# LeoIV/polyaxon

Hardware: AMD Instinct MI355X
Metric: HPO trials/hour (whole node) + wall-clock-to-target, ResNet-50 Hyperband sweep (higher is better)
Workload: dtype bf16

## Files before the change

polyaxon_amd/csrc/conv_gemm.hip:

```cpp
#include <hip/hip_runtime.h>

#include <stdint.h>

#include <type_traits>

namespace {

typedef __bf16 bf16x8 __attribute__((ext_vector_type(8)));
typedef short s16x4 __attribute__((ext_vector_type(4)));
typedef float f32x4 __attribute__((ext_vector_type(4)));
typedef uint32_t u32x4 __attribute__((ext_vector_type(4)));
typedef __attribute__((address_space(3))) void lds_void;
typedef __attribute__((address_space(1))) const void gbl_void;

constexpr int BK = 64;

struct ConvGeom {
    int H, W;
    int Hr, Wr;
    int C, S, ntaps;
    int Hc, Wc, OS, oph, opw;
    signed char offh[9], offw[9], btap[9];
    int tap_a[9], tap_b[9];
    uint32_t mWr, mHr;
// ... 24 lines not shown
        while (j < g.nw && g.wv[j] != g.offw[t]) ++j;
        if (j == g.nw) g.wv[g.nw++] = g.offw[t];
        g.pat[i * 3 + j] |= 1u << t;
    }
    g.mWr = div_magic(g.Wr);
    g.mHr = div_magic(g.Hr);
    return g;
}

struct BnBwd {
    const __bf16* x;
    const uint8_t* mask;
    const float* mean;
    const float* invstd;
    float* part;
    int part_ld, blk_off;
    int skip_h, skip_w;
};

struct BnDx {
    const __bf16* x;
    const uint8_t* mask;
    const float* coef;
    __bf16* dy;
};

struct BnApply {
    const __bf16* res;
    const float* sb;
    const float* rsb;
    __bf16* out;
    uint8_t* mask;
};

__device__ __forceinline__ void row_coords(int m, int Hr, int Wr, int& n, int& r, int& c) {
    const int q = m / Wr;
    c = m - q * Wr;
    n = q / Hr;
    r = q - n * Hr;
}

__device__ __forceinline__ void row_coords(int m, const ConvGeom& g, int& n, int& r, int& c) {
    const int q = g.mWr ? (int)__umulhi((uint32_t)m, g.mWr) : m;
    c = m - q * g.Wr;
    n = g.mHr ? (int)__umulhi((uint32_t)q, g.mHr) : q;
    r = q - n * g.Hr;
}

__device__ __forceinline__ size_t out_row(const ConvGeom& g, int m) {
    if (g.OS == 0) return (size_t)m;
    int n, r, c;
    row_coords(m, g.Hr, g.Wr, n, r, c);
    return ((size_t)n * g.Hc + r * g.OS + g.oph) * g.Wc + c * g.OS + g.opw;
}
constexpr int NTHREADS = 256;

template <int STEP>
__device__ __forceinline__ void wait_vm_stages(int stages) {
    if (stages >= 4 && 4 * STEP <= 63) asm volatile("s_waitcnt vmcnt(%0)" ::"n"(4 * STEP < 63 ? 4 * STEP : 63) : "memory");
    else if (stages >= 3) asm volatile("s_waitcnt vmcnt(%0)" ::"n"(3 * STEP) : "memory");
    else if (stages == 2) asm volatile("s_waitcnt vmcnt(%0)" ::"n"(2 * STEP) : "memory");
    else if (stages == 1) asm volatile("s_waitcnt vmcnt(%0)" ::"n"(STEP) : "memory");
    else asm volatile("s_waitcnt vmcnt(0)" ::: "memory");
}

__device__ __forceinline__ int xcd_remap(int bid, int nwg) {
    const int xcd = bid & 7, q = nwg >> 3, r = nwg & 7;
    const int base = xcd < r ? xcd * (q + 1) : r * (q + 1) + (xcd - r) * q;
    return base + (bid >> 3);
}

__device__ __forceinline__ void glds16(const void* g, void* l) {
    __builtin_amdgcn_global_load_lds((gbl_void*)g, (lds_void*)l, 16, 0, 0);
}

constexpr uint32_t OOB = 0x80000000u;

__device__ __forceinline__ __amdgpu_buffer_rsrc_t buf_rsrc(const void* base) {
    return __builtin_amdgcn_make_buffer_rsrc(const_cast<void*>(base), 0, (int)OOB, 0x00020000);
}

__device__ __forceinline__ void blds16(__amdgpu_buffer_rsrc_t r, uint32_t off, void* l) {
    __builtin_amdgcn_raw_ptr_buffer_load_lds(r, (lds_void*)l, 16, off, 0, 0, 0);
}

__device__ __forceinline__ uint32_t pack_bf16x2(float a, float b) {
    return (uint32_t)__builtin_bit_cast(uint16_t, (__bf16)a) | ((uint32_t)__builtin_bit_cast(uint16_t, (__bf16)b) << 16);
}

__device__ __forceinline__ int nt_swz(int row) { return (row >> 1) & 7; }

template <int BM, int BN, int WGM, int WGN, int MODE, int MINB = 2, int NBUF = 2, bool BWD = false, int NTH = NTHREADS,
          bool BNDX = false, int BNAP = 0>
__global__ void __launch_bounds__(NTH, MINB)
gemm_nt_kernel(const __bf16* __restrict__ A, const __bf16* __restrict__ B, __bf16* __restrict__ C,
               int M, int N, int K, int lda, int ldb, int ldc, float* __restrict__ stats, ConvGeom geo,
               const __bf16* __restrict__ D, int ldd, BnBwd bnr, const uint8_t* __restrict__ dmask, BnDx bd,
               BnApply ba) {
    constexpr bool CONV = MODE == 1, STEM = MODE == 2;
    constexpr bool PROD = BNDX || BNAP != 0;
    static_assert(BNAP >= 0 && BNAP <= 2 && !(BNDX && BNAP != 0), "one producer mode");
    static_assert(BNAP == 0 || (MODE == 0 && NBUF == 2 && !BWD && NTH == 256), "BNAP: dense double-buffered forward");
    static_assert(MODE >= 0 && MODE <= 2, "dense, gather or stem");
    static_assert(!BNDX || (MODE == 0 && NBUF == 2 && BWD && NTH == 256), "BNDX: dense double-buffered data gradient");
    constexpr int NW = NTH / 64;
    static_assert(WGM * WGN == NW, "one wave per wave tile");
    static_assert(NTH == 256 && NBUF >= 1 && NBUF <= 2, "4-wave kernels, one or two K stages");
    constexpr int WTM = BM / WGM, WTN = BN / WGN;
    constexpr int RM = WTM / 16, RN = WTN / 16;
    constexpr int A_BYTES = BM * BK * 2, B_BYTES = BN * BK * 2, STAGE = A_BYTES + B_BYTES;
    extern __shared__ __attribute__((aligned(16))) char smem[];

    const int tid = threadIdx.x, lane = tid & 63;
    const int wave = __builtin_amdgcn_readfirstlane(tid >> 6);
    const int ntn = N / BN, ntm = (M + BM - 1) / BM;
    const int id = xcd_remap(blockIdx.x, ntm * ntn);
    const int tn = id % ntn, tm = id / ntn;
    const int m0 = tm * BM, n0 = tn * BN;
    const int wm = wave / WGN, wn = wave % WGN;

    constexpr int AI = BM / (8 * NW), BI = BN / (8 * NW);
    int a_off[AI];
    uint32_t a_ok[AI];
#pragma unroll
    for (int i = 0; i < AI; ++i) {
        const int row = (i * NW + wave) * 8 + (lane >> 3);
        const int lc = (lane & 7) ^ nt_swz(row);
        const int gm = m0 + row;
        if constexpr (CONV) {
            int n, r, c;
            row_coords(gm, geo, n, r, c);
            const int ih0 = r * geo.S, iw0 = c * geo.S;
            a_off[i] = (((n * geo.H + ih0) * geo.W + iw0) * lda + lc * 8) * 2;
            uint32_t ok = 0;
#pragma unroll
            for (int hi = 0; hi < 3; ++hi) {
                const bool vh = hi < geo.nh && (unsigned)(ih0 + geo.hv[hi]) < (unsigned)geo.H;
#pragma unroll
                for (int wj = 0; wj < 3; ++wj) {
                    const bool vw = wj < geo.nw && (unsigned)(iw0 + geo.wv[wj]) < (unsigned)geo.W;
                    ok |= (vh && vw) ? geo.pat[hi * 3 + wj] : 0u;
                }
            }
            a_ok[i] = gm < M ? ok : 0u;
        } else if constexpr (STEM) {
            int n, r, c;
            row_coords(gm, geo, n, r, c);
            const int ih0 = 2 * r - 3, sc0 = c - 2;
            a_off[i] = ((n * geo.H + ih0) * geo.W + sc0) * 16;
            uint32_t ok = 0;
#pragma unroll
            for (int st = 0; st < 4; ++st) {
                const int t = st * 8 + lc;
                ok |= (t < 28 && (unsigned)(ih0 + (t >> 2)) < (unsigned)geo.H && (unsigned)(sc0 + (t & 3)) < (unsigned)geo.W)
                          ? 1u << st : 0u;
            }
            a_ok[i] = gm < M ? ok : 0u;
        } else {
            a_off[i] = (gm * lda + lc * 8) * 2;
            a_ok[i] = gm < M ? 1u : 0u;
        }
    }
    int b_off[BI];
#pragma unroll
    for (int i = 0; i < BI; ++i) {
        const int row = (i * NW + wave) * 8 + (lane >> 3);
// ... 813 lines not shown
        if (it + R2 < nu) issue(it + R2);
    }
    if (!lag) __builtin_amdgcn_s_barrier();
    asm volatile("s_waitcnt vmcnt(0) lgkmcnt(0)" ::: "memory");
    __syncthreads();
    float* red = (float*)smem;
    if (grp > 0) {
        float* dst = red + ((grp - 1) * GW + wg) * 4096 + lane;
#pragma unroll
        for (int a = 0; a < 4; ++a)
#pragma unroll
            for (int b = 0; b < 4; ++b)
#pragma unroll
                for (int r = 0; r < 4; ++r) dst[((a * 4 + b) * 4 + r) * 64] = acc[a][b][r];
    }
    __syncthreads();
    if (!ATOMIC && grp > 0) return;
    if (grp == 0) {
#pragma unroll 1
        for (int g = 1; g < KS; ++g) {
            const float* src = red + ((g - 1) * GW + wg) * 4096 + lane;
#pragma unroll
            for (int a = 0; a < 4; ++a)
#pragma unroll
                for (int b = 0; b < 4; ++b)
#pragma unroll
                    for (int r = 0; r < 4; ++r) acc[a][b][r] += src[((a * 4 + b) * 4 + r) * 64];
        }
    }
    if constexpr (ATOMIC) {
        __syncthreads();
        if (grp == 0) {
            float* t = red + wg * 4096;
#pragma unroll
            for (int a = 0; a < 4; ++a)
#pragma unroll
                for (int b = 0; b < 4; ++b)
#pragma unroll
                    for (int r = 0; r < 4; ++r) {
                        const int row = a * 16 + 4 * g4 + r, col = b * 16 + gi;
                        t[row * 64 + (col ^ (((row >> 2) & 3) << 4))] = acc[a][b][r];
                    }
        }
        __syncthreads();
#pragma unroll 4
        for (int j = wave; j < GW * 64; j += NW) {
            const int tw = j >> 6, row = j & 63;
            const float v = red[tw * 4096 + row * 64 + (lane ^ (((row >> 2) & 3) << 4))];
            float* dst = W + (size_t)(n10 + (tw / NB) * 64 + row) * ldc + n20 + (tw % NB) * 64 + lane;
            __hip_atomic_fetch_add(dst, v, __ATOMIC_RELAXED, __HIP_MEMORY_SCOPE_AGENT);
        }
        return;
    }
    float* slab = W + (size_t)slice * N1 * N2;
#pragma unroll
    for (int a = 0; a < 4; ++a)
#pragma unroll
        for (int b = 0; b < 4; ++b) {
            const int c2 = n20 + w2 * 64 + b * 16 + gi;
            const int r1 = n10 + w1 * 64 + a * 16 + 4 * g4;
#pragma unroll
            for (int r = 0; r < 4; ++r) slab[(size_t)(r1 + r) * N2 + c2] = acc[a][b][r];
        }
}

__global__ void weight_prep_kernel(const float* __restrict__ w, __bf16* __restrict__ wb, __bf16* __restrict__ wt,
                                   int cout, int cin) {
    __shared__ float tile[32][33];
    const int c0 = blockIdx.x * 32, o0 = blockIdx.y * 32;
    const int tx = threadIdx.x & 31, ty = threadIdx.x >> 5;
    for (int j = ty; j < 32; j += 8) {
        const int o = o0 + j, c = c0 + tx;
        float v = (o < cout && c < cin) ? w[(size_t)o * cin + c] : 0.f;
        tile[j][tx] = v;
        if (o < cout && c < cin) wb[(size_t)o * cin + c] = (__bf16)v;
    }
    __syncthreads();
    for (int j = ty; j < 32; j += 8) {
        const int c = c0 + j, o = o0 + tx;
        if (o < cout && c < cin) wt[(size_t)c * cout + o] = (__bf16)tile[tx][j];
    }
}

template <int NK>
__global__ void __launch_bounds__(512, 1)
bndx_wgrad_kernel(const __bf16* __restrict__ G, const __bf16* __restrict__ B, __bf16* __restrict__ C, int M, int ldb,
                  int ldc, const __bf16* __restrict__ D, int ldd, BnBwd bnr, const uint8_t* __restrict__ dmask, BnDx bd,
                  const __bf16* __restrict__ Xin, float* __restrict__ dW, int lddw) {
    constexpr int BM = 256, BN = 64, NW = 8, K = NK * BK;
    constexpr int A_BYTES = BM * BK * 2, B_BYTES = BN * BK * 2, STAGE = A_BYTES + B_BYTES;
    constexpr int XOFF = 2 * STAGE;
    constexpr int AI = BM / (8 * NW);
    extern __shared__ __attribute__((aligned(16))) char smem[];

    const int ntm = (M + BM - 1) / BM;
    if ((int)blockIdx.x >= ntm) return;
    const int tid = threadIdx.x, lane = tid & 63;
    const int wave = __builtin_amdgcn_readfirstlane(tid >> 6);
    const int fr = lane & 15, fq = lane >> 4;

    const int srow = wave * 8 + (lane >> 3);
    const int lc8 = ((lane & 7) ^ tr_swz<128>(srow)) * 8;
    const uint32_t b_off = (uint32_t)((srow * ldb + ((lane & 7) ^ nt_swz(srow)) * 8) * 2);
    const __amdgpu_buffer_rsrc_t rg = buf_rsrc(G), rb = buf_rsrc(B), rx = buf_rsrc(bd.x), rc = buf_rsrc(bd.coef),
                                 rxi = buf_rsrc(Xin);
    uint32_t e_off[AI];
    u32x4 gq[AI], xq[AI];
    uint32_t mq[AI];
    u32x4 cf[6];
    auto set_tile = [&](int m0) {
#pragma unroll
        for (int i = 0; i < AI; ++i) {
            const int gm = m0 + i * 64 + srow;
            e_off[i] = gm < M ? (uint32_t)((gm * K + lc8) * 2) : OOB;
        }
    };
    auto stage_x = [&](int m0) {
#pragma unroll
        for (int i = 0; i < AI; ++i) {
            const int gm = m0 + i * 64 + srow;
            blds16(rxi, gm < M ? (uint32_t)((gm * BN + lc8) * 2) : OOB, smem + XOFF + (i * NW + wave) * 1024);
        }
    };
    auto stage_b = [&](int buf, int k0) { blds16(rb, b_off + (uint32_t)(k0 * 2), smem + buf * STAGE + A_BYTES + wave * 1024); };
    auto load_a = [&](int k0) {
#pragma unroll
        for (int i = 0; i < AI; ++i) {
            gq[i] = __builtin_amdgcn_raw_buffer_load_b128(rg, (int)e_off[i], k0 * 2, 0);
            xq[i] = __builtin_amdgcn_raw_buffer_load_b128(rx, (int)e_off[i], k0 * 2, 0);
        }
        if (bd.mask != nullptr) {
            const __amdgpu_buffer_rsrc_t rm = buf_rsrc(bd.mask);
#pragma unroll
            for (int i = 0; i < AI; ++i)
                mq[i] = __builtin_amdgcn_raw_buffer_load_b8(rm, (int)(e_off[i] == OOB ? OOB : e_off[i] >> 4), k0 >> 3, 0);
        } else {
#pragma unroll
            for (int i = 0; i < AI; ++i) mq[i] = 0xffu;
        }
#pragma unroll
        for (int r = 0; r < 3; ++r) {
            cf[2 * r] = __builtin_amdgcn_raw_buffer_load_b128(rc, lc8 * 4, (r * K + k0) * 4, 0);
            cf[2 * r + 1] = __builtin_amdgcn_raw_buffer_load_b128(rc, lc8 * 4 + 16, (r * K + k0) * 4, 0);
        }
    };
    auto xform_a = [&](int buf) {
        char* base = smem + buf * STAGE;
        const float* ca = (const float*)&cf[0];
        const float* cb = (const float*)&cf[2];
        const float* cd = (const float*)&cf[4];
#pragma unroll
        for (int i = 0; i < AI; ++i) {
            const uint32_t* pg = (const uint32_t*)&gq[i];
            const uint32_t* px = (const uint32_t*)&xq[i];
            u32x4 o;
            uint32_t* po = (uint32_t*)&o;
            const uint32_t mb = mq[i];
#pragma unroll
            for (int j = 0; j < 4; ++j) {
                const float g0 = (mb >> (2 * j)) & 1u ? __uint_as_float(pg[j] << 16) : 0.f;
                const float g1 = (mb >> (2 * j + 1)) & 1u ? __uint_as_float(pg[j] & 0xffff0000u) : 0.f;
                const float x0 = __uint_as_float(px[j] << 16), x1 = __uint_as_float(px[j] & 0xffff0000u);
                const float o0 = fmaf(ca[2 * j], g0, fmaf(cb[2 * j], x0, cd[2 * j]));
                const float o1 = fmaf(ca[2 * j + 1], g1, fmaf(cb[2 * j + 1], x1, cd[2 * j + 1]));
                po[j] = pack_bf16x2(o0, o1);
            }
            if (e_off[i] == OOB) o = u32x4{0u, 0u, 0u, 0u};
            *(u32x4*)(base + (i * NW + wave) * 1024 + lane * 16) = o;
        }
    };

    f32x4 accw[NK][2];
#pragma unroll
    for (int a = 0; a < NK; ++a) accw[a][0] = accw[a][1] = f32x4{0.f, 0.f, 0.f, 0.f};
    const int kt4 = wave >> 1, nt2 = (wave & 1) * 2;
    const int trow = 8 * fq + (fr >> 2), tcol = 4 * (fr & 3);
    auto tr_off = [&](int col) {
        return (uint32_t)(trow * 128 + (((col >> 3) ^ tr_swz<128>(trow)) << 4) + ((col >> 2) & 1) * 8);
    };
    const uint32_t wa_off = tr_off(kt4 * 16 + tcol), wx_off0 = tr_off(nt2 * 16 + tcol), wx_off1 = tr_off(nt2 * 16 + 16 + tcol);

    constexpr int CROW = BN * 2 + 16, CHUNKS = BN / 8, RSTEP = 256 / CHUNKS, ITERS = BM / RSTEP;
    char* const ep = smem + STAGE;
    const bool bnr_on = bnr.part != nullptr, d_on = D != nullptr;

    int tm = blockIdx.x;
    set_tile(tm * BM);
    stage_x(tm * BM);
    load_a(0);
    stage_b(0, 0);
    for (; tm < ntm; tm += gridDim.x) {
        const int m0 = tm * BM;
        f32x4 acc[4][2];
#pragma unroll
        for (int a = 0; a < 4; ++a) acc[a][0] = acc[a][1] = f32x4{0.f, 0.f, 0.f, 0.f};
        xform_a(0);
        asm volatile("s_waitcnt vmcnt(0)" ::: "memory");
        __syncthreads();
#pragma unroll
        for (int kt = 0; kt < NK; ++kt) {
            const int cur = kt & 1;
            if (kt + 1 < NK) {
                load_a((kt + 1) * BK);
                stage_b(cur ^ 1, (kt + 1) * BK);
            }
            const char* As = smem + cur * STAGE;
            const char* Bs = As + A_BYTES;
#pragma unroll
            for (int kk = 0; kk < 2; ++kk) {
                bf16x8 fa[4], fb[2];
#pragma unroll
                for (int rn = 0; rn < 4; ++rn) {
                    const int row = rn * 16 + fr;
                    fa[rn] = *(const bf16x8*)(Bs + row * 128 + (((kk * 4 + fq) ^ nt_swz(row)) << 4));
                }
#pragma unroll
                for (int rm = 0; rm < 2; ++rm) {
                    const int row = wave * 32 + rm * 16 + fr;
                    fb[rm] = *(const bf16x8*)(As + row * 128 + (((kk * 4 + fq) ^ tr_swz<128>(row)) << 4));
                }
#pragma unroll
                for (int rn = 0; rn < 4; ++rn)
#pragma unroll
                    for (int rm = 0; rm < 2; ++rm)
                        acc[rn][rm] = __builtin_amdgcn_mfma_f32_16x16x32_bf16(fa[rn], fb[rm], acc[rn][rm], 0, 0, 0);
            }
            const uint32_t sa_ = lds_addr(As) + wa_off;
            const uint32_t sx_[2] = {lds_addr(smem + XOFF) + wx_off0, lds_addr(smem + XOFF) + wx_off1};
            auto dw_steps = [&](auto msc) {
                constexpr int O = decltype(msc)::value * 32 * 128;
                s16x4 alo[2], ahi[2], xlo[2][2], xhi[2][2];
                alo[0] = ds_tr_o<O>(sa_);
                ahi[0] = ds_tr_o<O + 512>(sa_);
                alo[1] = ds_tr_o<O + 4096>(sa_);
                ahi[1] = ds_tr_o<O + 4608>(sa_);
#pragma unroll
                for (int j = 0; j < 2; ++j) {
                    xlo[0][j] = ds_tr_o<O>(sx_[j]);
                    xhi[0][j] = ds_tr_o<O + 512>(sx_[j]);
                    xlo[1][j] = ds_tr_o<O + 4096>(sx_[j]);
                    xhi[1][j] = ds_tr_o<O + 4608>(sx_[j]);
                }
                asm volatile("s_waitcnt lgkmcnt(0)"
                             : "+v"(alo[0]), "+v"(ahi[0]), "+v"(alo[1]), "+v"(ahi[1]), "+v"(xlo[0][0]), "+v"(xhi[0][0]),
                               "+v"(xlo[0][1]), "+v"(xhi[0][1]), "+v"(xlo[1][0]), "+v"(xhi[1][0]), "+v"(xlo[1][1]),
                               "+v"(xhi[1][1]));
#pragma unroll
                for (int u = 0; u < 2; ++u) {
                    const bf16x8 fw = __builtin_bit_cast(bf16x8, __builtin_shufflevector(alo[u], ahi[u], 0, 1, 2, 3, 4, 5, 6, 7));
#pragma unroll
                    for (int j = 0; j < 2; ++j) {
                        const bf16x8 fx =
                            __builtin_bit_cast(bf16x8, __builtin_shufflevector(xlo[u][j], xhi[u][j], 0, 1, 2, 3, 4, 5, 6, 7));
                        accw[kt][j] = __builtin_amdgcn_mfma_f32_16x16x32_bf16(fw, fx, accw[kt][j], 0, 0, 0);
                    }
                }
            };
            dw_steps(std::integral_constant<int, 0>{});
            dw_steps(std::integral_constant<int, 2>{});
            dw_steps(std::integral_constant<int, 4>{});
            dw_steps(std::integral_constant<int, 6>{});
            __builtin_amdgcn_sched_barrier(0);
            if (kt + 1 < NK) xform_a(cur ^ 1);
            asm volatile("s_waitcnt vmcnt(0)" ::: "memory");
            __syncthreads();
        }
        const int tnext = tm + gridDim.x;
        if (tnext < ntm) {
            set_tile(tnext * BM);
            stage_x(tnext * BM);
            load_a(0);
            stage_b(0, 0);
        }
        const int rows = min(BM, M - m0);
        int te = tid;
        asm volatile("" : "+v"(te));
        const int cc = te % CHUNKS, ch0 = cc * 8;
        const bool ep_thread = te < 256;
#pragma unroll
        for (int rm = 0; rm < 2; ++rm) {
            const int ml = wave * 32 + rm * 16 + fr;
#pragma unroll
            for (int rn = 0; rn < 4; ++rn) {
                const f32x4 v = acc[rn][rm];
                uint2 packed;
                packed.x = pack_bf16x2(v[0], v[1]);
                packed.y = pack_bf16x2(v[2], v[3]);
                *(uint2*)(ep + ml * CROW + (rn * 16 + fq * 4) * 2) = packed;
            }
        }
        __syncthreads();
        {
            constexpr int AIT = BM / 64;
            const int ra0 = te / CHUNKS;
            int orow[AIT];
            uint4 dpre[AIT];
            uint32_t dmpre[AIT];
#pragma unroll
            for (int i = 0; i < AIT; ++i) orow[i] = min(m0 + ra0 + i * 64, M - 1);
            if (d_on) {
#pragma unroll
                for (int i = 0; i < AIT; ++i) dpre[i] = *(const uint4*)(D + (size_t)orow[i] * ldd + ch0);
                if (dmask != nullptr) {
#pragma unroll
                    for (int i = 0; i < AIT; ++i) dmpre[i] = dmask[((size_t)orow[i] * ldd + ch0) >> 3];
                }
            }
#pragma unroll
            for (int i = 0; i < AIT; ++i) {
                const int r = ra0 + i * 64;
                if (r >= rows) break;
                uint4 v = *(const uint4*)(ep + r * CROW + cc * 16);
                if (d_on) {
                    uint32_t* pv = (uint32_t*)&v;
                    const uint32_t* pd = (const uint32_t*)&dpre[i];
                    const uint32_t db = dmask != nullptr ? dmpre[i] : 0xffu;
#pragma unroll
                    for (int j = 0; j < 4; ++j) {
                        const float d0 = (db >> (2 * j)) & 1u ? __uint_as_float(pd[j] << 16) : 0.f;
                        const float d1 = (db >> (2 * j + 1)) & 1u ? __uint_as_float(pd[j] & 0xffff0000u) : 0.f;
                        const float lo = __uint_as_float(pv[j] << 16) + d0;
                        const float hi = __uint_as_float(pv[j] & 0xffff0000u) + d1;
                        pv[j] = pack_bf16x2(lo, hi);
                    }
                    if (bnr_on) *(uint4*)(ep + r * CROW + cc * 16) = v;
                }
                *(uint4*)(C + (size_t)orow[i] * ldc + ch0) = v;
            }
        }
        float sa[8], sb[8];
        if (bnr_on) {
            __syncthreads();
            if (ep_thread) {
                const int r0 = te / CHUNKS;
                float mu[8], is[8];
#pragma unroll
                for (int k = 0; k < 8; ++k) {
                    sa[k] = sb[k] = 0.f;
                    mu[k] = bnr.mean[ch0 + k];
                    is[k] = bnr.invstd[ch0 + k];
                }
#pragma unroll
                for (int h = 0; h < 2; ++h) {
                    constexpr int HI = ITERS / 2;
                    asm volatile("" ::: "memory");
                    uint4 xpre[HI];
                    uint32_t mpre[HI];
#pragma unroll
                    for (int i = 0; i < HI; ++i) {
                        const size_t e = (size_t)min(m0 + r0 + (h * HI + i) * RSTEP, M - 1) * ldc + ch0;
                        xpre[i] = *(const uint4*)(bnr.x + e);
                        mpre[i] = bnr.mask != nullptr ? bnr.mask[e >> 3] : 0xffu;
                    }
                    if (bnr.skip_w > 0) {
#pragma unroll
                        for (int i = 0; i < HI; ++i) {
                            const int gm = m0 + r0 + (h * HI + i) * RSTEP, q = gm / bnr.skip_w;
                            if (((gm - q * bnr.skip_w) | (q % bnr.skip_h)) % 2 == 0) mpre[i] = 0u;
                        }
                    }
#pragma unroll
                    for (int i = 0; i < HI; ++i) {
                        const int r = r0 + (h * HI + i) * RSTEP;
                        if (r >= rows) break;
                        const uint4 v = *(const uint4*)(ep + r * CROW + cc * 16);
                        const uint32_t mb = mpre[i];
                        const uint32_t* pv = (const uint32_t*)&v;
                        const uint32_t* px = (const uint32_t*)&xpre[i];
#pragma unroll
                        for (int j = 0; j < 4; ++j) {
                            const float g0 = (mb >> (2 * j)) & 1u ? __uint_as_float(pv[j] << 16) : 0.f;
                            const float g1 = (mb >> (2 * j + 1)) & 1u ? __uint_as_float(pv[j] & 0xffff0000u) : 0.f;
                            const float x0 = __uint_as_float(px[j] << 16), x1 = __uint_as_float(px[j] & 0xffff0000u);
                            sa[2 * j] += g0;
                            sa[2 * j + 1] += g1;
                            sb[2 * j] = fmaf(g0, (x0 - mu[2 * j]) * is[2 * j], sb[2 * j]);
                            sb[2 * j + 1] = fmaf(g1, (x1 - mu[2 * j + 1]) * is[2 * j + 1], sb[2 * j + 1]);
                        }
                    }
                }
            }
        }
        if (bnr_on) {
            float* red = (float*)ep;
            __syncthreads();
            if (ep_thread) {
#pragma unroll
                for (int k = 0; k < 8; ++k) {
                    red[te * 17 + k] = sa[k];
                    red[te * 17 + 8 + k] = sb[k];
                }
            }
            __syncthreads();
            if (te < CHUNKS * 16) {
                const int c = te % CHUNKS, v = te / CHUNKS;
                float sum = 0.f;
#pragma unroll 4
                for (int j = 0; j < RSTEP; ++j) sum += red[(j * CHUNKS + c) * 17 + v];
                float* pa = bnr.part + (size_t)(bnr.blk_off + tm) * ldc;
                float* pb = bnr.part + (size_t)(bnr.part_ld + bnr.blk_off + tm) * ldc;
                if (v < 8) pa[c * 8 + v] = sum;
                else pb[c * 8 + v - 8] = sum;
            }
        }
    }
    asm volatile("s_waitcnt vmcnt(0)" ::: "memory");
    __syncthreads();
    float* red = (float*)smem;
    static_assert(K * 256 <= 2 * STAGE, "the flush image fits the stage buffers");
#pragma unroll
    for (int kt = 0; kt < NK; ++kt)
#pragma unroll
        for (int j = 0; j < 2; ++j)
#pragma unroll
            for (int r = 0; r < 4; ++r) {
                const int row = kt * 64 + kt4 * 16 + 4 * fq + r, col = (nt2 + j) * 16 + fr;
                red[row * 64 + (col ^ (((row >> 2) & 3) << 4))] = accw[kt][j][r];
            }
    __syncthreads();
#pragma unroll 4
    for (int row = wave; row < K; row += NW) {
        const float v = red[row * 64 + (lane ^ (((row >> 2) & 3) << 4))];
        __hip_atomic_fetch_add(dW + (size_t)row * lddw + lane, v, __ATOMIC_RELAXED, __HIP_MEMORY_SCOPE_AGENT);
    }
}

template <typename KernelT>
int set_lds(KernelT k, int bytes) {
    return hipFuncSetAttribute((const void*)k, hipFuncAttributeMaxDynamicSharedMemorySize, bytes) == hipSuccess ? 0
                                                                                                                 : -2;
}

template <int BM, int BN, int WGM, int WGN, int CONV = 0, int NBUF = 2>
int launch_nt(const void* A, const void* B, void* C, int M, int N, int K, int lda, int ldb, int ldc, float* stats,
              hipStream_t s, ConvGeom geo = {}, const void* D = nullptr, int ldd = 0, BnBwd bnr = {},
              const uint8_t* dmask = nullptr) {
    constexpr int NTH = NTHREADS;
    constexpr int TILE = BM * (BN * 2 + 16), RED = NTH * 17 * 4;
    constexpr int EPI = TILE > RED ? TILE : RED;
    constexpr int KLOOP = NBUF * (BM + BN) * BK * 2;
    constexpr int LDS = KLOOP > EPI ? KLOOP : EPI;
    static_assert(NBUF >= 1 && NBUF <= 2, "one or two K stages");
    static_assert(NBUF == 1 || EPI <= KLOOP, "epilogue staging must fit the k-loop LDS");
    static_assert(LDS <= 160 * 1024, "LDS");
    constexpr int PER_CU = (160 * 1024) / LDS;
    constexpr int CAP = CONV != 0 && BN == 64 ? 3 : 4;
    constexpr int MIN_F = NBUF == 1 ? (PER_CU < CAP ? PER_CU : CAP) : 2, MIN_B = MIN_F;
    auto kf = gemm_nt_kernel<BM, BN, WGM, WGN, CONV, MIN_F, NBUF, false, NTH>;
    auto kb = gemm_nt_kernel<BM, BN, WGM, WGN, CONV, MIN_B, NBUF, true, NTH>;
    static int attr = set_lds(kf, LDS) | set_lds(kb, LDS);
    if (attr) return attr;
    const bool bwd = D != nullptr || bnr.part != nullptr;
    if (bwd && stats != nullptr) return -1;
    auto k = bwd ? kb : kf;
    const int nwg = ((M + BM - 1) / BM) * (N / BN);
    hipLaunchKernelGGL(k, dim3(nwg), dim3(NTH), LDS, s, (const __bf16*)A, (const __bf16*)B, (__bf16*)C, M, N,
                       K, lda, ldb, ldc, stats, geo, (const __bf16*)D, ldd, bnr, dmask, BnDx{}, BnApply{});
    return hipGetLastError() == hipSuccess ? 0 : -3;
}

template <int BM, int BN, int WGM, int WGN, bool BNDX, int BNAP>
int launch_nt_prod(const void* A, const BnDx& bd, const BnApply& ba, const void* B, void* C, int M, int N, int K,
                   int ldb, int ldc, float* stats, hipStream_t s, const void* D = nullptr, int ldd = 0, BnBwd bnr = {},
                   const uint8_t* dmask = nullptr) {
    constexpr int TILE = BM * (BN * 2 + 16), RED = NTHREADS * 17 * 4;
    constexpr int LDS = 2 * (BM + BN) * BK * 2;
    static_assert(TILE <= LDS && RED <= LDS && LDS <= 80 * 1024, "epilogue staging fits; 2 blocks per CU");
    static_assert(BNDX != (BNAP != 0), "exactly one producer mode");
    auto k = gemm_nt_kernel<BM, BN, WGM, WGN, 0, 2, 2, BNDX, NTHREADS, BNDX, BNAP>;
    static int attr = set_lds(k, LDS);
    if (attr) return attr;
    const int nwg = ((M + BM - 1) / BM) * (N / BN);
    hipLaunchKernelGGL(k, dim3(nwg), dim3(NTHREADS), LDS, s, (const __bf16*)A, (const __bf16*)B, (__bf16*)C, M, N, K, K,
                       ldb, ldc, stats, ConvGeom{}, (const __bf16*)D, ldd, bnr, dmask, bd, ba);
    return hipGetLastError() == hipSuccess ? 0 : -3;
}

template <int NK>
int launch_bndx_wgrad(const void* g, const BnDx& bd, const void* Wt, void* C, int M, int ldb, int ldc, const void* D,
                      int ldd, const BnBwd& bnr, const uint8_t* dmask, const void* x_in, float* dW, int lddw, int blocks,
                      hipStream_t s) {
    constexpr int LDS = 2 * (256 + 64) * BK * 2 + 256 * 64 * 2;
    static_assert(LDS <= 160 * 1024, "LDS");
    auto k = bndx_wgrad_kernel<NK>;
    static int attr = set_lds(k, LDS);
    if (attr) return attr;
    int grid = blocks;
    if (grid <= 0) {
        int dev = 0, cus = 0;
        if (hipGetDevice(&dev) != hipSuccess ||
            hipDeviceGetAttribute(&cus, hipDeviceAttributeMultiprocessorCount, dev) != hipSuccess || cus <= 0)
            return -3;
        const int ntm = (M + 255) / 256;
        grid = cus < ntm ? cus : ntm;
    }
    hipLaunchKernelGGL(k, dim3(grid), dim3(512), LDS, s, (const __bf16*)g, (const __bf16*)Wt, (__bf16*)C, M, ldb, ldc,
                       (const __bf16*)D, ldd, bnr, dmask, bd, (const __bf16*)x_in, dW, lddw);
    return hipGetLastError() == hipSuccess ? 0 : -3;
}


inline bool nt_single(bool conv, int K, int nwg) { return nwg >= 768 || (!conv && K == BK); }

inline int nt_plan(bool conv, int M, int N, int K) {
    const int bm = N % 128 == 0 ? 128 : 256, bn = N % 128 == 0 ? 128 : 64;
    return bm + 1000 * (nt_single(conv, K, ((M + bm - 1) / bm) * (N / bn)) ? 1 : 2);
}

struct TnPlan { int kchunk, slices, groups, per_group, blocks, bn1, bn2; };

inline void tn_tile(int N1, int N2, int& bn1, int& bn2) {
    bn1 = N1 % 128 == 0 ? 128 : 64;
    bn2 = N2 % 128 == 0 ? 128 : 64;
}

inline void plan_reducer(TnPlan& p, long plane) {
    const long total4 = plane / 4;
    int blocks = (int)((total4 + 255) / 256);
    if (blocks > 2048) blocks = 2048;
    int groups = 1024 / blocks;
    if (groups > p.slices / 8) groups = p.slices / 8;
    if (groups < 1) groups = 1;
    const int per_group = (p.slices + groups - 1) / groups;
    p.groups = (p.slices + per_group - 1) / per_group;
    p.per_group = per_group;
    p.blocks = blocks;
}

inline long plan_slabs(const TnPlan& p) { return p.slices + (p.groups > 1 ? p.groups : 0); }

constexpr int g_tn_bpc_big = 3, g_tn_bpc_mid = 1;
constexpr long g_tn_slab_bytes = 16l << 20;

inline TnPlan tn_plan(int M, int N1, int N2, int num_cus, int bpc = 0) {
    int bn1, bn2;
    tn_tile(N1, N2, bn1, bn2);
    const int ntiles = (N1 / bn1) * (N2 / bn2);
    const long plane = (long)N1 * N2;
    const int bpc_eff = bpc > 0 ? bpc : (M >= 400000 ? g_tn_bpc_big : M >= 150000 ? g_tn_bpc_mid : 1);
    int slices = (bpc_eff * (num_cus > 0 ? num_cus : 256)) / ntiles;
    const int by_depth = M / (4 * BK);
    const int by_bytes = (int)(g_tn_slab_bytes / (plane * 4));
    if (slices > by_depth) slices = by_depth;
    if (slices > by_bytes) slices = by_bytes;
    if (slices < 1) slices = 1;
    int kchunk = (M + slices - 1) / slices;
    kchunk = ((kchunk + BK - 1) / BK) * BK;
    TnPlan p{kchunk, (M + kchunk - 1) / kchunk, 1, 1, 0, bn1, bn2};
    plan_reducer(p, plane);
    return p;
}

template <int BN1, int BN2, int WG1, int WG2, int CONV, int NST, int BKT = BK>
int launch_tn_st(const void* A, const void* B, float* W, int M, int N1, int N2, int lda, int ldb, const TnPlan& plan,
                 hipStream_t s, const ConvGeom& geo) {
    constexpr int LDS = NST * BKT * (BN1 + BN2) * 2;
    static_assert(LDS <= 160 * 1024, "LDS ring exceeds the CU's LDS");
    auto k = gemm_tn_kernel<BN1, BN2, WG1, WG2, CONV, NST, BKT>;
    static int attr = set_lds(k, LDS);
    if (attr) return attr;
    const int ntiles = (N1 / BN1) * (N2 / BN2);
    hipLaunchKernelGGL(k, dim3(ntiles * plan.slices), dim3(NTHREADS), LDS, s, (const __bf16*)A, (const __bf16*)B, W,
                       M, N1, N2, lda, ldb, plan.kchunk, geo);
    return hipGetLastError() == hipSuccess ? 0 : -3;
}
// ... 90 lines not shown
template <int CONV>
int dispatch_tn2(const V2Cfg& c, const void* A, const void* B, float* W, int M, int N1, int N2, int lda, int ldb,
                 const TnPlan& plan, hipStream_t s, const ConvGeom& geo, bool atomic = false, int ldc = 0) {
    if constexpr (CONV == 2) {
        if (c.na == 1 && c.nb == 4 && c.ks == 2)
            return atomic ? launch_tn2<1, 4, 2, 2, true>(A, B, W, M, N1, N2, lda, ldb, plan, s, geo, ldc)
                          : launch_tn2<1, 4, 2, 2, false>(A, B, W, M, N1, N2, lda, ldb, plan, s, geo, ldc);
        return -1;
    } else {
#define PLX_TN2(a, b, k) \
    if (c.na == a && c.nb == b && c.ks == k) \
        return atomic ? launch_tn2<a, b, k, CONV, true>(A, B, W, M, N1, N2, lda, ldb, plan, s, geo, ldc) \
                      : launch_tn2<a, b, k, CONV, false>(A, B, W, M, N1, N2, lda, ldb, plan, s, geo, ldc);
        PLX_TN2(2, 2, 2) PLX_TN2(1, 4, 2) PLX_TN2(1, 3, 2) PLX_TN2(1, 2, 4) PLX_TN2(1, 1, 8) PLX_TN2(4, 1, 2)
        PLX_TN2(2, 1, 4)
#undef PLX_TN2
        return -1;
    }
}

template <int BN1, int BN2, int WG1, int WG2, int CONV = 0>
int launch_tn(const void* A, const void* B, float* W, int M, int N1, int N2, int lda, int ldb, const TnPlan& plan,
              hipStream_t s, ConvGeom geo = {}) {
    return launch_tn_st<BN1, BN2, WG1, WG2, CONV, 2>(A, B, W, M, N1, N2, lda, ldb, plan, s, geo);
}

}

extern "C" {

int plx_gemm_nt_rows_per_block(int N) { return N % 128 == 0 ? 128 : 256; }

int plx_gemm_nt(const void* A, const void* B, void* C, int M, int N, int K, int lda, int ldb, int ldc,
                float* stats, const void* D, int ldd, const uint8_t* dmask, const BnBwd* bnr, void* stream) {
    if (M <= 0 || N % 64 || K % BK || lda % 8 || ldb % 8 || ldc % 8 || (D != nullptr && ldd % 8)) return -1;
    if (dmask != nullptr && (D == nullptr || ldd != N)) return -1;
    if (bnr != nullptr && (ldc != N || bnr->part == nullptr)) return -1;
    const BnBwd b = bnr != nullptr ? *bnr : BnBwd{};
    hipStream_t s = (hipStream_t)stream;
    switch (nt_plan(false, M, N, K)) {
        case 1128:
            return launch_nt<128, 128, 2, 2, false, 1>(A, B, C, M, N, K, lda, ldb, ldc, stats, s, {}, D, ldd, b, dmask);
        case 2128:
            return launch_nt<128, 128, 2, 2>(A, B, C, M, N, K, lda, ldb, ldc, stats, s, {}, D, ldd, b, dmask);
        case 1256:
            return launch_nt<256, 64, 4, 1, false, 1>(A, B, C, M, N, K, lda, ldb, ldc, stats, s, {}, D, ldd, b, dmask);
        default:
            return launch_nt<256, 64, 4, 1>(A, B, C, M, N, K, lda, ldb, ldc, stats, s, {}, D, ldd, b, dmask);
    }
}

int plx_gemm_nt_plan(int M, int N, int K, int conv) {
    if (M <= 0 || N <= 0 || N % 64 || K <= 0 || K % BK) return -1;
    return nt_plan(conv != 0, M, N, K);
}

int plx_gemm_nt_bndx(const void* g, const void* x, const uint8_t* mask, const float* coef, void* dy, const void* Wt,
                     void* C, int M, int N, int K, int ldb, int ldc, const void* D, int ldd, const uint8_t* dmask,
                     const BnBwd* bnr, void* stream) {
    if (M <= 0 || N % 64 || K % BK || ldb % 8 || ldc % 8 || (D != nullptr && ldd % 8)) return -1;
    if (g == nullptr || x == nullptr || coef == nullptr || dy == nullptr || dy == g || dy == x) return -1;
    if ((long)M * K >= (1l << 30)) return -1;
    if (dmask != nullptr && (D == nullptr || ldd != N)) return -1;
    if (bnr != nullptr && (ldc != N || bnr->part == nullptr)) return -1;
    const BnBwd b = bnr != nullptr ? *bnr : BnBwd{};
    const BnDx bd{(const __bf16*)x, mask, coef, (__bf16*)dy};
    hipStream_t s = (hipStream_t)stream;
    if (N % 128 == 0)
        return launch_nt_prod<128, 128, 2, 2, true, 0>(g, bd, {}, Wt, C, M, N, K, ldb, ldc, nullptr, s, D, ldd, b, dmask);
    return launch_nt_prod<256, 64, 4, 1, true, 0>(g, bd, {}, Wt, C, M, N, K, ldb, ldc, nullptr, s, D, ldd, b, dmask);
}

int plx_gemm_nt_bndx_wgrad(const void* g, const void* x, const uint8_t* mask, const float* coef, void* dy,
                           const void* Wt, void* C, int M, int N, int K, int ldb, int ldc, const void* D, int ldd,
                           const uint8_t* dmask, const BnBwd* bnr, const void* x_in, float* dW, int lddw, int blocks,
                           void* stream) {
    (void)dy;
    if (M <= 0 || N != 64 || K % BK || K < BK || K > 4 * BK || ldb % 8 || ldc % 8 || (D != nullptr && ldd % 8)) return -1;
    if (g == nullptr || x == nullptr || coef == nullptr || x_in == nullptr || dW == nullptr || lddw < N || blocks < 0)
        return -1;
    if ((long)M * K >= (1l << 30)) return -1;
    if (dmask != nullptr && (D == nullptr || ldd != N)) return -1;
    if (bnr != nullptr && (ldc != N || bnr->part == nullptr)) return -1;
    const BnBwd b = bnr != nullptr ? *bnr : BnBwd{};
    const BnDx bd{(const __bf16*)x, mask, coef, nullptr};
    hipStream_t s = (hipStream_t)stream;
    switch (K / BK) {
        case 1: return launch_bndx_wgrad<1>(g, bd, Wt, C, M, ldb, ldc, D, ldd, b, dmask, x_in, dW, lddw, blocks, s);
        case 2: return launch_bndx_wgrad<2>(g, bd, Wt, C, M, ldb, ldc, D, ldd, b, dmask, x_in, dW, lddw, blocks, s);
        case 3: return launch_bndx_wgrad<3>(g, bd, Wt, C, M, ldb, ldc, D, ldd, b, dmask, x_in, dW, lddw, blocks, s);
        default: return launch_bndx_wgrad<4>(g, bd, Wt, C, M, ldb, ldc, D, ldd, b, dmask, x_in, dW, lddw, blocks, s);
    }
}

int plx_gemm_nt_bnapply(const void* x, const void* res, const float* sb, const float* rsb, void* out, uint8_t* mask,
                        const void* W, void* C, int M, int N, int K, int ldb, int ldc, float* stats, void* stream) {
    if (M <= 0 || N % 64 || K % BK || ldb % 8 || ldc % 8) return -1;
    if (x == nullptr || res == nullptr || sb == nullptr || out == nullptr || mask == nullptr || out == x || out == res)
        return -1;
    if ((long)M * K >= (1l << 30)) return -1;
    const BnApply ba{(const __bf16*)res, sb, rsb, (__bf16*)out, mask};
    hipStream_t s = (hipStream_t)stream;
    if (N % 128 == 0)
        return rsb != nullptr ? launch_nt_prod<128, 128, 2, 2, false, 2>(x, {}, ba, W, C, M, N, K, ldb, ldc, stats, s)
                              : launch_nt_prod<128, 128, 2, 2, false, 1>(x, {}, ba, W, C, M, N, K, ldb, ldc, stats, s);
    return rsb != nullptr ? launch_nt_prod<256, 64, 4, 1, false, 2>(x, {}, ba, W, C, M, N, K, ldb, ldc, stats, s)
                          : launch_nt_prod<256, 64, 4, 1, false, 1>(x, {}, ba, W, C, M, N, K, ldb, ldc, stats, s);
}

int plx_tn_plan_slices(int M, int N1, int N2, int num_cus, int v2) {
    if (M <= 0 || N1 % 64 || N2 % 64) return -1;
    return v2 ? tn2_plan(M, N1, N2, num_cus, v2_cfg(N1, N2)).slices : tn_plan(M, N1, N2, num_cus).slices;
}

void plx_set_tn2_c64(int on) { g_tn2_c64 = on ? 1 : 0; }

void plx_set_tn_atomic(int on) { g_tn_atomic = on ? 1 : 0; }

int plx_get_tn_atomic() { return g_tn_atomic; }

void plx_set_tn2_stem(int mode) { g_tn2_stem = mode < 0 ? 0 : (mode > 2 ? 2 : mode); }

void plx_set_tn_v2(int on, int lds_kb) {
    g_tn_v2 = on < 0 ? 0 : (on > 2 ? 2 : on);
    if (lds_kb > 0) g_tn2_lds_kb = lds_kb <= 64 ? 64 : 128;
}

long plx_gemm_tn_workspace(int M, int N1, int N2, int num_cus) {
    if (M <= 0 || N1 % 64 || N2 % 64) return -1;
    const long a = plan_slabs(tn_plan(M, N1, N2, num_cus));
    const long b = plan_slabs(tn2_plan(M, N1, N2, num_cus, v2_cfg(N1, N2)));
    return (a > b ? a : b) * N1 * N2;
}

}

namespace {
template <int CONV>
int run_tn(const void* A, const void* B, float* C, float* ws, int M, int N1, int N2, int lda, int ldb, int ldc,
           int num_cus, int accumulate, hipStream_t s, ConvGeom geo, int bpc = 0) {
    const V2Cfg cfg = v2_cfg(N1, N2);
    const bool six = cfg.na == 1 && cfg.nb == 3;
    const bool v2 = CONV == 2 ? g_tn2_stem > 0
                              : (g_tn_v2 == 1 || (g_tn_v2 == 2 && CONV != 0)) && (!six || g_tn2_c64);
    const TnPlan plan = v2 ? tn2_plan(M, N1, N2, num_cus, cfg, CONV == 2 && g_tn2_stem == 1 ? kStemV2Bpc : 0)
                           : tn_plan(M, N1, N2, num_cus, bpc);
    int rc;
    if (v2 && g_tn_atomic) {
        if (!accumulate && hipMemset2DAsync(C, (size_t)ldc * 4, 0, (size_t)N2 * 4, N1, s) != hipSuccess) return -3;
        return dispatch_tn2<CONV>(cfg, A, B, C, M, N1, N2, lda, ldb, plan, s, geo, true, ldc);
    }
    if (v2)
        rc = dispatch_tn2<CONV>(cfg, A, B, ws, M, N1, N2, lda, ldb, plan, s, geo);
    else if (N1 % 128 == 0 && N2 % 128 == 0)
        rc = launch_tn<128, 128, 2, 2, CONV>(A, B, ws, M, N1, N2, lda, ldb, plan, s, geo);
    else if (N1 % 128 == 0)
        rc = launch_tn<128, 64, 4, 1, CONV>(A, B, ws, M, N1, N2, lda, ldb, plan, s, geo);
    else if (N2 % 128 == 0)
        rc = launch_tn<64, 128, 1, 4, CONV>(A, B, ws, M, N1, N2, lda, ldb, plan, s, geo);
    else
        rc = launch_tn<64, 64, 2, 2, CONV>(A, B, ws, M, N1, N2, lda, ldb, plan, s, geo);
    if (rc) return rc;
    const long plane = (long)N1 * N2;
    const float* slabs = ws;
    int nslabs = plan.slices;
    if (plan.groups > 1) {
// ... 316 lines not shown
```

Before: 13190.

## Prefetch epilogue operands into LDS and overlap next-tile loads in bndx wgrad kernel

Restructures the software pipeline of the fused BN-dx/weight-grad kernel. The residual D, the BN input x and the masks are now staged into LDS with async buffer-to-LDS loads during the last K step, instead of being read from global memory in the epilogue. Next-tile A loads are issued earlier with partial vmcnt waits, and the x/B staging for the next tile is moved after the reduction. The epilogue uses a swizzled LDS layout, and BN mean/invstd are cached in LDS. This enlarges the LDS footprint and adds alignment preconditions, and the hand-set vmcnt counts are fragile.

```diff
diff --git a/polyaxon_amd/csrc/conv_gemm.hip b/polyaxon_amd/csrc/conv_gemm.hip
--- a/polyaxon_amd/csrc/conv_gemm.hip
+++ b/polyaxon_amd/csrc/conv_gemm.hip
@@ -130,6 +130,16 @@
 
 __device__ __forceinline__ void blds16(__amdgpu_buffer_rsrc_t r, uint32_t off, void* l) {
     __builtin_amdgcn_raw_ptr_buffer_load_lds(r, (lds_void*)l, 16, off, 0, 0, 0);
+}
+
+__device__ __forceinline__ void blds4(__amdgpu_buffer_rsrc_t r, uint32_t off, void* l) {
+    __builtin_amdgcn_raw_ptr_buffer_load_lds(r, (lds_void*)l, 4, off, 0, 0, 0);
+}
+
+__device__ __forceinline__ void lds_barrier() {
+    asm volatile("s_waitcnt lgkmcnt(0)" ::: "memory");
+    __builtin_amdgcn_s_barrier();
+    asm volatile("" ::: "memory");
 }
 
 __device__ __forceinline__ uint32_t pack_bf16x2(float a, float b) {
@@ -1109,6 +1119,8 @@
     }
 }
 
+constexpr int BNDX_WGRAD_LDS = 2 * (256 + 64) * BK * 2 + 2 * 256 * 64 * 2 + 2 * 256 * 8 + 2 * 64 * 4;
+
 template <int NK>
 __global__ void __launch_bounds__(512, 1)
 bndx_wgrad_kernel(const __bf16* __restrict__ G, const __bf16* __restrict__ B, __bf16* __restrict__ C, int M, int ldb,
@@ -1118,6 +1130,10 @@
     constexpr int A_BYTES = BM * BK * 2, B_BYTES = BN * BK * 2, STAGE = A_BYTES + B_BYTES;
     constexpr int XOFF = 2 * STAGE;
     constexpr int AI = BM / (8 * NW);
+    constexpr int EXOFF = XOFF + BM * BN * 2, EMOFF = EXOFF + BM * BN * 2, DMOFF = EMOFF + BM * BN / 8,
+                  STOFF = DMOFF + BM * BN / 8;
+    static_assert(STOFF + 2 * BN * 4 == BNDX_WGRAD_LDS, "LDS layout");
+    constexpr int LAST = (NK - 1) & 1;
     extern __shared__ __attribute__((aligned(16))) char smem[];
 
     const int ntm = (M + BM - 1) / BM;
@@ -1150,6 +1166,31 @@
         }
     };
     auto stage_b = [&](int buf, int k0) { blds16(rb, b_off + (uint32_t)(k0 * 2), smem + buf * STAGE + A_BYTES + wave * 1024); };
+    const bool bnr_on = bnr.part != nullptr, d_on = D != nullptr;
+    auto fetch_epi = [&](int m0) {
+        if (d_on) {
+            const __amdgpu_buffer_rsrc_t rd = buf_rsrc(D);
+#pragma unroll
+            for (int i = 0; i < AI; ++i) {
+                const int gm = m0 + i * 64 + srow;
+                blds16(rd, gm < M ? (uint32_t)((gm * ldd + (lane & 7) * 8) * 2) : OOB,
+                       smem + (LAST ^ 1) * STAGE + (i * NW + wave) * 1024);
+            }
+        }
+        if (bnr_on) {
+            const __amdgpu_buffer_rsrc_t rbx = buf_rsrc(bnr.x);
+#pragma unroll
+            for (int i = 0; i < AI; ++i) {
+                const int gm = m0 + i * 64 + srow;
+                blds16(rbx, gm < M ? (uint32_t)((gm * ldc + (lane & 7) * 8) * 2) : OOB,
+                       smem + EXOFF + (i * NW + wave) * 1024);
+            }
+        }
+        const int mrow = m0 + wave * 32 + (lane >> 1);
+        const uint32_t m_off = mrow < M ? (uint32_t)(mrow * (BN / 8) + (lane & 1) * 4) : OOB;
+        if (d_on && dmask != nullptr) blds4(buf_rsrc(dmask), m_off, smem + DMOFF + wave * 256);
+        if (bnr_on && bnr.mask != nullptr) blds4(buf_rsrc(bnr.mask), m_off, smem + EMOFF + wave * 256);
+    };
     auto load_a = [&](int k0) {
 #pragma unroll
         for (int i = 0; i < AI; ++i) {
@@ -1207,17 +1248,20 @@
     };
     const uint32_t wa_off = tr_off(kt4 * 16 + tcol), wx_off0 = tr_off(nt2 * 16 + tcol), wx_off1 = tr_off(nt2 * 16 + 16 + tcol);
 
-    constexpr int CROW = BN * 2 + 16, CHUNKS = BN / 8, RSTEP = 256 / CHUNKS, ITERS = BM / RSTEP;
-    char* const ep = smem + STAGE;
-    const bool bnr_on = bnr.part != nullptr, d_on = D != nullptr;
-
+    constexpr int CHUNKS = BN / 8, RSTEP = 256 / CHUNKS, ITERS = BM / RSTEP;
+    char* const ep = smem + LAST * STAGE;
+    char* const dimg = smem + (LAST ^ 1) * STAGE;
+    auto ep_at = [&](int row, int chunk) { return ep + row * 128 + ((chunk ^ (row & 7)) << 4); };
+    static_assert(256 * 17 * 4 <= A_BYTES, "the reduction staging fits the A region");
+
+    if (bnr_on && tid < 2 * BN) ((float*)(smem + STOFF))[tid] = tid < BN ? bnr.mean[tid] : bnr.invstd[tid - BN];
     int tm = blockIdx.x;
     set_tile(tm * BM);
     stage_x(tm * BM);
     load_a(0);
     stage_b(0, 0);
     for (; tm < ntm; tm += gridDim.x) {
-        const int m0 = tm * BM;
+        const int m0 = tm * BM, tnext = tm + gridDim.x;
         f32x4 acc[4][2];
 #pragma unroll
         for (int a = 0; a < 4; ++a) acc[a][0] = acc[a][1] = f32x4{0.f, 0.f, 0.f, 0.f};
@@ -1227,10 +1271,7 @@
 #pragma unroll
         for (int kt = 0; kt < NK; ++kt) {
             const int cur = kt & 1;
-            if (kt + 1 < NK) {
-                load_a((kt + 1) * BK);
-                stage_b(cur ^ 1, (kt + 1) * BK);
-            }
+            if (kt == 0 && NK > 1) load_a(BK);
             const char* As = smem + cur * STAGE;
             const char* Bs = As + A_BYTES;
 #pragma unroll
@@ -1252,6 +1293,9 @@
                     for (int rm = 0; rm < 2; ++rm)
                         acc[rn][rm] = __builtin_amdgcn_mfma_f32_16x16x32_bf16(fa[rn], fb[rm], acc[rn][rm], 0, 0, 0);
             }
+            __builtin_amdgcn_sched_barrier(0);
+            if (kt + 1 < NK) stage_b(cur ^ 1, (kt + 1) * BK);
+            else fetch_epi(m0);
             const uint32_t sa_ = lds_addr(As) + wa_off;
             const uint32_t sx_[2] = {lds_addr(smem + XOFF) + wx_off0, lds_addr(smem + XOFF) + wx_off1};
             auto dw_steps = [&](auto msc) {
@@ -1288,16 +1332,29 @@
             dw_steps(std::integral_constant<int, 4>{});
             dw_steps(std::integral_constant<int, 6>{});
             __builtin_amdgcn_sched_barrier(0);
-            if (kt + 1 < NK) xform_a(cur ^ 1);
-            asm volatile("s_waitcnt vmcnt(0)" ::: "memory");
-            __syncthreads();
-        }
-        const int tnext = tm + gridDim.x;
-        if (tnext < ntm) {
+            if (kt + 1 < NK) {
+                xform_a(cur ^ 1);
+                bool ahead = true;
+                if (kt + 2 < NK) {
+                    load_a((kt + 2) * BK);
+                } else if (tnext < ntm) {
+                    set_tile(tnext * BM);
+                    load_a(0);
+                } else {
+                    ahead = false;
+                }
+                if (!ahead) asm volatile("s_waitcnt vmcnt(0)" ::: "memory");
+                else if (bd.mask != nullptr) asm volatile("s_waitcnt vmcnt(18)" ::: "memory");
+                else asm volatile("s_waitcnt vmcnt(14)" ::: "memory");
+                lds_barrier();
+            } else {
+                asm volatile("s_waitcnt vmcnt(0)" ::: "memory");
+                __syncthreads();
+            }
+        }
+        if (NK == 1 && tnext < ntm) {
             set_tile(tnext * BM);
-            stage_x(tnext * BM);
             load_a(0);
-            stage_b(0, 0);
         }
         const int rows = min(BM, M - m0);
         int te = tid;
@@ -1313,35 +1370,23 @@
                 uint2 packed;
                 packed.x = pack_bf16x2(v[0], v[1]);
                 packed.y = pack_bf16x2(v[2], v[3]);
-                *(uint2*)(ep + ml * CROW + (rn * 16 + fq * 4) * 2) = packed;
+                *(uint2*)(ep_at(ml, rn * 2 + (fq >> 1)) + (fq & 1) * 8) = packed;
             }
         }
         __syncthreads();
         {
             constexpr int AIT = BM / 64;
             const int ra0 = te / CHUNKS;
-            int orow[AIT];
-            uint4 dpre[AIT];
-            uint32_t dmpre[AIT];
-#pragma unroll
-            for (int i = 0; i < AIT; ++i) orow[i] = min(m0 + ra0 + i * 64, M - 1);
-            if (d_on) {
-#pragma unroll
-                for (int i = 0; i < AIT; ++i) dpre[i] = *(const uint4*)(D + (size_t)orow[i] * ldd + ch0);
-                if (dmask != nullptr) {
-#pragma unroll
-                    for (int i = 0; i < AIT; ++i) dmpre[i] = dmask[((size_t)orow[i] * ldd + ch0) >> 3];
-                }
-            }
 #pragma unroll
             for (int i = 0; i < AIT; ++i) {
                 const int r = ra0 + i * 64;
                 if (r >= rows) break;
-                uint4 v = *(const uint4*)(ep + r * CROW + cc * 16);
+                uint4 v = *(const uint4*)ep_at(r, cc);
                 if (d_on) {
                     uint32_t* pv = (uint32_t*)&v;
-                    const uint32_t* pd = (const uint32_t*)&dpre[i];
-                    const uint32_t db = dmask != nullptr ? dmpre[i] : 0xffu;
+                    const uint4 dq = *(const uint4*)(dimg + i * (NW * 1024) + te * 16);
+                    const uint32_t* pd = (const uint32_t*)&dq;
+                    const uint32_t db = dmask != nullptr ? (uint32_t)(uint8_t)smem[DMOFF + r * CHUNKS + cc] : 0xffu;
 #pragma unroll
                     for (int j = 0; j < 4; ++j) {
                         const float d0 = (db >> (2 * j)) & 1u ? __uint_as_float(pd[j] << 16) : 0.f;
@@ -1350,9 +1395,9 @@
                         const float hi = __uint_as_float(pv[j] & 0xffff0000u) + d1;
                         pv[j] = pack_bf16x2(lo, hi);
                     }
-                    if (bnr_on) *(uint4*)(ep + r * CROW + cc * 16) = v;
+                    if (bnr_on) *(uint4*)ep_at(r, cc) = v;
                 }
-                *(uint4*)(C + (size_t)orow[i] * ldc + ch0) = v;
+                *(uint4*)(C + (size_t)(m0 + r) * ldc + ch0) = v;
             }
         }
         float sa[8], sb[8];
@@ -1360,50 +1405,36 @@
             __syncthreads();
             if (ep_thread) {
                 const int r0 = te / CHUNKS;
+                const float* st = (const float*)(smem + STOFF);
                 float mu[8], is[8];
 #pragma unroll
                 for (int k = 0; k < 8; ++k) {
                     sa[k] = sb[k] = 0.f;
-                    mu[k] = bnr.mean[ch0 + k];
-                    is[k] = bnr.invstd[ch0 + k];
+                    mu[k] = st[ch0 + k];
+                    is[k] = st[BN + ch0 + k];
                 }
 #pragma unroll
-                for (int h = 0; h < 2; ++h) {
-                    constexpr int HI = ITERS / 2;
-                    asm volatile("" ::: "memory");
-                    uint4 xpre[HI];
-                    uint32_t mpre[HI];
-#pragma unroll
-                    for (int i = 0; i < HI; ++i) {
-                        const size_t e = (size_t)min(m0 + r0 + (h * HI + i) * RSTEP, M - 1) * ldc + ch0;
-                        xpre[i] = *(const uint4*)(bnr.x + e);
-                        mpre[i] = bnr.mask != nullptr ? bnr.mask[e >> 3] : 0xffu;
+                for (int it = 0; it < ITERS; ++it) {
+                    const int r = r0 + it * RSTEP;
+                    if (r >= rows) break;
+                    const uint4 v = *(const uint4*)ep_at(r, cc);
+                    const uint4 xv = *(const uint4*)(smem + EXOFF + r * 128 + cc * 16);
+                    uint32_t mb = bnr.mask != nullptr ? (uint32_t)(uint8_t)smem[EMOFF + r * CHUNKS + cc] : 0xffu;
+                    if (bnr.skip_w > 0) {
+                        const int gm = m0 + r, q = gm / bnr.skip_w;
+                        if (((gm - q * bnr.skip_w) | (q % bnr.skip_h)) % 2 == 0) mb = 0u;
                     }
-                    if (bnr.skip_w > 0) {
-#pragma unroll
-                        for (int i = 0; i < HI; ++i) {
-                            const int gm = m0 + r0 + (h * HI + i) * RSTEP, q = gm / bnr.skip_w;
-                            if (((gm - q * bnr.skip_w) | (q % bnr.skip_h)) % 2 == 0) mpre[i] = 0u;
-                        }
-                    }
-#pragma unroll
-                    for (int i = 0; i < HI; ++i) {
-                        const int r = r0 + (h * HI + i) * RSTEP;
-                        if (r >= rows) break;
-                        const uint4 v = *(const uint4*)(ep + r * CROW + cc * 16);
-                        const uint32_t mb = mpre[i];
-                        const uint32_t* pv = (const uint32_t*)&v;
-                        const uint32_t* px = (const uint32_t*)&xpre[i];
-#pragma unroll
-                        for (int j = 0; j < 4; ++j) {
-                            const float g0 = (mb >> (2 * j)) & 1u ? __uint_as_float(pv[j] << 16) : 0.f;
-                            const float g1 = (mb >> (2 * j + 1)) & 1u ? __uint_as_float(pv[j] & 0xffff0000u) : 0.f;
-                            const float x0 = __uint_as_float(px[j] << 16), x1 = __uint_as_float(px[j] & 0xffff0000u);
-                            sa[2 * j] += g0;
-                            sa[2 * j + 1] += g1;
-                            sb[2 * j] = fmaf(g0, (x0 - mu[2 * j]) * is[2 * j], sb[2 * j]);
-                            sb[2 * j + 1] = fmaf(g1, (x1 - mu[2 * j + 1]) * is[2 * j + 1], sb[2 * j + 1]);
-                        }
+                    const uint32_t* pv = (const uint32_t*)&v;
+                    const uint32_t* px = (const uint32_t*)&xv;
+#pragma unroll
+                    for (int j = 0; j < 4; ++j) {
+                        const float g0 = (mb >> (2 * j)) & 1u ? __uint_as_float(pv[j] << 16) : 0.f;
+                        const float g1 = (mb >> (2 * j + 1)) & 1u ? __uint_as_float(pv[j] & 0xffff0000u) : 0.f;
+                        const float x0 = __uint_as_float(px[j] << 16), x1 = __uint_as_float(px[j] & 0xffff0000u);
+                        sa[2 * j] += g0;
+                        sa[2 * j + 1] += g1;
+                        sb[2 * j] = fmaf(g0, (x0 - mu[2 * j]) * is[2 * j], sb[2 * j]);
+                        sb[2 * j + 1] = fmaf(g1, (x1 - mu[2 * j + 1]) * is[2 * j + 1], sb[2 * j + 1]);
                     }
                 }
             }
@@ -1429,6 +1460,11 @@
                 if (v < 8) pa[c * 8 + v] = sum;
                 else pb[c * 8 + v - 8] = sum;
             }
+        }
+        if ((NK & 1) || !bnr_on) __syncthreads();
+        if (tnext < ntm) {
+            stage_x(tnext * BM);
+            stage_b(0, 0);
         }
     }
     asm volatile("s_waitcnt vmcnt(0)" ::: "memory");
@@ -1507,7 +1543,7 @@
 int launch_bndx_wgrad(const void* g, const BnDx& bd, const void* Wt, void* C, int M, int ldb, int ldc, const void* D,
                       int ldd, const BnBwd& bnr, const uint8_t* dmask, const void* x_in, float* dW, int lddw, int blocks,
                       hipStream_t s) {
-    constexpr int LDS = 2 * (256 + 64) * BK * 2 + 256 * 64 * 2;
+    constexpr int LDS = BNDX_WGRAD_LDS;
     static_assert(LDS <= 160 * 1024, "LDS");
     auto k = bndx_wgrad_kernel<NK>;
     static int attr = set_lds(k, LDS);
@@ -1764,6 +1800,8 @@
     if ((long)M * K >= (1l << 30)) return -1;
     if (dmask != nullptr && (D == nullptr || ldd != N)) return -1;
     if (bnr != nullptr && (ldc != N || bnr->part == nullptr)) return -1;
+    if (D != nullptr && ((long)M * ldd >= (1l << 30) || ((uintptr_t)D & 15))) return -1;
+    if (((uintptr_t)dmask & 3) || (bnr != nullptr && (((uintptr_t)bnr->mask & 3) || ((uintptr_t)bnr->x & 15)))) return -1;
     const BnBwd b = bnr != nullptr ? *bnr : BnBwd{};
     const BnDx bd{(const __bf16*)x, mask, coef, nullptr};
     hipStream_t s = (hipStream_t)stream;
```

Result: no change. 13220 (median of 6 runs) (+0.3%).
